# alessandroragano/nomad

Measured on AMD Instinct MI355X. Metric: clips/sec embedded + NxM NOMAD distances, 16kHz x 4s batches, higher is better.
Workload: dtype f32

## Files before the change

### nomad_amd/csrc/nomad_ctx.hip.h

```cpp
#pragma once
#include <hip/hip_runtime.h>

#include <algorithm>
#include <cmath>
#include <cstdarg>
#include <cstdio>
#include <cstdlib>
#include <cstring>
#include <atomic>
#include <mutex>
#include <string>
#include <vector>

#include "../../include/nomad_hip.h"

#include "dtypes.hip.h"
#include "gemm_f32.hip.h"

#define NOMAD_INTERNAL __attribute__((visibility("hidden")))

using namespace nomad;

inline thread_local char g_err[512] = "";

namespace {

int fail(int code, const char* fmt, ...) {
    va_list ap;
    va_start(ap, fmt);
    vsnprintf(g_err, sizeof(g_err), fmt, ap);
    va_end(ap);
    return code;
}

#define HIP_TRY(expr)                                                                        \
    do {                                                                                     \
        hipError_t _e = (expr);                                                              \
        if (_e != hipSuccess) return fail(NOMAD_ERR_HIP, "%s: %s", #expr, hipGetErrorString(_e)); \
    } while (0)

constexpr int kConvK[7] = {10, 3, 3, 3, 3, 2, 2};
constexpr int kConvS[7] = {5, 2, 2, 2, 2, 2, 2};
constexpr int kSplitKLayersMaxM = 4096;
constexpr size_t kSplitKPartFloats = (size_t)4 * 512 * 64 * 64;
constexpr long long kPairScratchDoubles = 1 << 21;
constexpr int kEventChunk = 8192;
const int* const kNoInts = nullptr;
const hipStream_t kNoStream = reinterpret_cast<hipStream_t>(~uintptr_t(0));

}

struct LayerDev {
    float *qkv_w, *qkv_b, *o_w, *o_b, *ln1_w, *ln1_b, *fc1_w, *fc1_b, *fc2_w, *fc2_b, *ln2_w, *ln2_b;
};


struct Tuning {
    bool splitk_lnb_fuse = true;
    bool splitk_ln_fuse = true;
    bool splitk_posconv = true;
    bool splitk_layers = true;
    bool f32_plain_epi = true;
    bool f32_lean = true, f32_direct_epi = true, f32_skew = true, f32_res_ahead = true;
    int f32_mixed = 1;
    int f32_mixed_m1 = 0;
    int f32_mixed_slots = 0;
    double f32_mixed_min = 0.05, f32_mixed_max = 0.70;
    bool f32_mixed_prefer = false;
    bool f32_quant_tile = true;
    double f32_quant_penalty = 0.0;
    bool f32_longk_33 = false;
    int f32_mid_tile = 31;
    bool f32_attn_vt4 = true;
    bool f32_attn_struct_loads = false;
    bool bf16_posconv_slab = true;
    int bf16_attn_dma = 2;
    int bf16_attn_v3 = 2;
    int bf16_attn_tail = 0;
    int bf16_ln_rows = 4;
    bool bf16_conv0_mfma = true;
    bool bf16_conv0_gelu_erf = false;
    int p8_min_tiles = 256;
    bool p8_nt_stores = true;
    int p8_rpre = 3;
    bool x3_plain_epi = true;
    bool p8_three_b = true;
    int p8_n192 = 0;
    bool p9 = true;
    bool p9_res = true;
    bool p9_share = false;
    bool p9_tail_split = false;
    int p9_short = 1;
    bool attn_bwd_small = true;
    bool p9_wl = false;
    bool p9_late = true;
    int p9_skew = 0;
    int concurrent_parts = 1;
};

#ifdef NOMAD_DIAG
static void tuning_from_env(Tuning& t) {
    auto geti = [](const char* n, int d) { const char* e = getenv(n); return e ? atoi(e) : d; };
    auto getb = [](const char* n, bool d) { const char* e = getenv(n); return e ? atoi(e) != 0 : d; };
    auto getd = [](const char* n, double d) { const char* e = getenv(n); return e ? atof(e) : d; };
    t.splitk_ln_fuse = getb("NOMAD_SPLITK_LN", t.splitk_ln_fuse);
    t.splitk_posconv = getb("NOMAD_SPLITK_POSCONV", t.splitk_posconv);
    t.splitk_layers = getb("NOMAD_SPLITK_LAYERS", t.splitk_layers);
    t.f32_plain_epi = getb("NOMAD_F32_PLAIN_EPI", t.f32_plain_epi);
    t.f32_lean = getb("NOMAD_F32_LEAN", t.f32_lean);
    t.f32_direct_epi = getb("NOMAD_F32_DIRECT_EPI", t.f32_direct_epi);
    t.f32_skew = getb("NOMAD_F32_SKEW", t.f32_skew);
    t.f32_res_ahead = getb("NOMAD_F32_RES_AHEAD", t.f32_res_ahead);
    t.f32_mixed = geti("NOMAD_F32_MIXED", t.f32_mixed);
    t.f32_mixed_m1 = geti("NOMAD_F32_MIXED_M1", t.f32_mixed_m1);
    t.f32_mixed_slots = geti("NOMAD_F32_MIXED_SLOTS", t.f32_mixed_slots);
    t.f32_mixed_min = getd("NOMAD_F32_MIXED_MIN", t.f32_mixed_min);
    t.f32_mixed_max = getd("NOMAD_F32_MIXED_MAX", t.f32_mixed_max);
    t.f32_mixed_prefer = getb("NOMAD_F32_MIXED_PREFER", t.f32_mixed_prefer);
    t.f32_quant_tile = getb("NOMAD_F32_QUANT_TILE", t.f32_quant_tile);
    t.f32_quant_penalty = getd("NOMAD_F32_QUANT_PENALTY", t.f32_quant_penalty);
    t.f32_longk_33 = getb("NOMAD_F32_LONGK_33", t.f32_longk_33);
    t.f32_mid_tile = geti("NOMAD_F32_MID_TILE", t.f32_mid_tile);
    t.bf16_attn_dma = geti("NOMAD_BF16_ATTN_DMA", t.bf16_attn_dma);
    t.f32_attn_struct_loads = geti("NOMAD_F32_ATTN_STRUCT_LOADS", t.f32_attn_struct_loads) != 0;
    t.bf16_posconv_slab = geti("NOMAD_BF16_POSCONV_SLAB", t.bf16_posconv_slab) != 0;
    t.bf16_attn_v3 = geti("NOMAD_BF16_ATTN_V3", t.bf16_attn_v3);
    t.bf16_attn_tail = geti("NOMAD_BF16_ATTN_TAIL", t.bf16_attn_tail);
    t.bf16_ln_rows = geti("NOMAD_BF16_LN_ROWS", t.bf16_ln_rows);
    t.bf16_conv0_mfma = getb("NOMAD_BF16_CONV0_MFMA", t.bf16_conv0_mfma);
    t.p8_min_tiles = geti("NOMAD_BF16_8PHASE_MIN_TILES", t.p8_min_tiles);
    t.p8_nt_stores = getb("NOMAD_BF16_NT_STORES", t.p8_nt_stores);
    t.p8_rpre = geti("NOMAD_BF16_RPRE", t.p8_rpre);
    t.x3_plain_epi = getb("NOMAD_X3_PLAIN_EPI", t.x3_plain_epi);
    t.p8_three_b = getb("NOMAD_BF16_B3", t.p8_three_b);
    t.p8_n192 = geti("NOMAD_BF16_N192", t.p8_n192);
    t.p9 = getb("NOMAD_BF16_P9", t.p9);
    t.p9_tail_split = getb("NOMAD_BF16_P9_TAIL", t.p9_tail_split);
    t.p9_share = getb("NOMAD_BF16_P9_SHARE", t.p9_share);
    t.p9_res = getb("NOMAD_BF16_P9_RES", t.p9_res);
    t.p9_short = geti("NOMAD_BF16_P9_SHORT", t.p9_short);
    t.p9_skew = geti("NOMAD_BF16_P9_SKEW", t.p9_skew);
    t.p9_late = getb("NOMAD_BF16_P9_LATE", t.p9_late);
    t.p9_wl = getb("NOMAD_BF16_P9_WL", t.p9_wl);
    t.splitk_lnb_fuse = getb("NOMAD_SPLITK_LNB", t.splitk_lnb_fuse);
    t.f32_attn_vt4 = getb("NOMAD_F32_ATTN_VT4", t.f32_attn_vt4);
    t.bf16_conv0_gelu_erf = getb("NOMAD_BF16_CONV0_GELU_ERF", t.bf16_conv0_gelu_erf);
    t.attn_bwd_small = getb("NOMAD_ATTN_BWD_SMALL", t.attn_bwd_small);
}
#endif

struct nomad_ctx {
    int device = 0;
    int num_cus = 256;
    Tuning tune;
    bool keep = false;
    float* conv0_w = nullptr;
    float* conv_w[7] = {};
    float *gn_w = nullptr, *gn_b = nullptr, *fln_w = nullptr, *fln_b = nullptr;
    float *proj_w = nullptr, *proj_b = nullptr;
    float *pos_w = nullptr, *pos_b = nullptr;
    float *eln_w = nullptr, *eln_b = nullptr;
    LayerDev layers[NOMAD_NUM_LAYERS] = {};
    float *emb_w = nullptr, *emb_b = nullptr;
    float* splitk_part = nullptr;
    float* splitk_cur = nullptr;
    bool splitk_ok = false;
    struct PendingLn {
        const float* gamma = nullptr;
        const float* beta = nullptr;
        float* out = nullptr;
        float* out2 = nullptr;
        bool armed = false, done = false;
// ... 86 lines not shown
        c->p_fl[cls] += flops;
        c->p_n[cls] += 1;
        if (cls2 >= 0) {
            c->p_fl[cls2] += flops;
            c->p_n[cls2] += 1;
        }
        slot = c->ev_used;
        c->ev_class[slot / 2] = cls | ((cls2 + 1) << 8);
        c->ev_used += 2;
        (void)hipEventRecord(c->ev[slot], s);
    }
    ~Scope() {
        if (slot >= 0) (void)hipEventRecord(c->ev[slot + 1], s);
    }
};

RowMap plain_map(int M, int ld) { return RowMap{0, 0, M > 0 ? M : 1, ld}; }

int occ_pad(int occ, int lds) {
    if (occ <= 0) return 0;
    const int budget = (160 * 1024 / occ) & ~255;
    return budget > lds ? budget - lds : 0;
}

GemmParams dense(const float* A, int lda, const float* W, const float* bias, const float* R, float* C, int M, int N,
                 int K, int gelu) {
    GemmParams p{};
    p.A = A;
    p.amap = plain_map(M, lda);
    p.kchunk = K;
    p.kstride = 0;
    p.W = W;
    p.ldw = K;
    p.C = C;
    p.cmap = plain_map(M, N);
    p.bias = bias;
    p.R = R;
    p.rmap = plain_map(M, N);
    p.M = M;
    p.N = N;
    p.K = K;
    p.n_valid = N;
    p.gelu = gelu;
    return p;
}

}

NOMAD_INTERNAL int run_gemm(nomad_ctx* c, GemmParams p, int groups, int tile, hipStream_t s, int occ = 0);
NOMAD_INTERNAL int gemm_f32_dispatch(nomad_ctx* c, GemmParams p, int groups, int tile, hipStream_t s, int occ);
NOMAD_INTERNAL hipError_t gemm_f32_n48_split(const GemmParams& q, int groups, hipStream_t s, int S);
NOMAD_INTERNAL int pick_tile(const nomad_ctx* c, int M, int N, int K);
NOMAD_INTERNAL int mixed_split_rows(const nomad_ctx* c, int M, int N);
NOMAD_INTERNAL int run_gemm_bf16(nomad_ctx* c, GemmParams p, int groups, hipStream_t s, int tile = -1);
#ifdef NOMAD_DIAG
NOMAD_INTERNAL int gemm_f32_timeline_read(unsigned long long* out_host, int n);
NOMAD_INTERNAL int gemm_bf16_timeline_read(unsigned long long* out_host, int n);
#endif
```

### nomad_amd/csrc/nomad_gemm_f32.hip

```cpp
#include "nomad_ctx.hip.h"

int gemm_f32_dispatch(nomad_ctx* c, GemmParams p, int groups, int tile, hipStream_t s, int occ) {
    if (tile == 29 && occ == 0) occ = 4;
    const double flops = 2.0 * p.M * (double)p.n_valid * p.K * groups;
    Scope sc(c, s, NOMAD_K_GEMM, flops, tile == 33 ? NOMAD_K_GEMM_BIG : ((tile == 34 || tile == 31 || tile == 48) ? NOMAD_K_GEMM_FINE : -1));
    hipError_t e;
    if (c->gemm_x3 && tile == 48 && p.N == 64)
        tile = 37;
    if (c->gemm_x3 && (tile == 31 || tile == 34 || tile == 37) && p.N % 128 == 0 &&
        (long long)((p.M + 127) / 128) * (p.N / 128) >= 512)
        tile = 20;
    const bool plain_cr = c->tune.f32_plain_epi && p.c_colblk == 0 && p.cmap.clip_rows >= p.M && !p.cmap.pref &&
                          (!p.R || (p.rmap.clip_rows >= p.M && !p.rmap.pref)) && (!p.DG || (p.dgmap.clip_rows >= p.M && !p.dgmap.pref));
    if (c->gemm_x3 && plain_cr && (tile == 20 || tile == 31 || tile == 34 || tile == 37)) {
        constexpr int T = 16 | 32;
        switch (tile) {
            case 20: e = launch_gemm_glds<128, 128, 32, 2, 2, 2, false, 12 | T, true>(p, groups, s, occ_pad(occ, GldsCfg<128, 128, 32, 2, 2>::LDS_BYTES)); break;
            case 31: e = launch_gemm_glds<128, 128, 32, 4, 2, 2, false, 12 | T, true>(p, groups, s, occ_pad(occ, GldsCfg<128, 128, 32, 4, 2>::LDS_BYTES)); break;
            case 34: e = launch_gemm_glds<128, 64, 32, 4, 2, 3, false, 12 | T, true>(p, groups, s); break;
            default: e = launch_gemm_glds<64, 64, 32, 2, 2, 3, false, 12 | T, true>(p, groups, s); break;
        }
        if (e != hipSuccess) return fail(NOMAD_ERR_HIP, "gemm (bf16x3 products) launch: %s", hipGetErrorString(e));
        return 0;
    }
    if (c->gemm_x3 && (tile == 20 || tile == 31 || tile == 33 || tile == 34 || tile == 37)) {
        switch (tile) {
            case 20: e = launch_gemm_glds<128, 128, 32, 2, 2, 2, false, 12, true>(p, groups, s, occ_pad(occ, GldsCfg<128, 128, 32, 2, 2>::LDS_BYTES)); break;
            case 31: e = launch_gemm_glds<128, 128, 32, 4, 2, 2, false, 12, true>(p, groups, s, occ_pad(occ, GldsCfg<128, 128, 32, 4, 2>::LDS_BYTES)); break;
            case 33: e = launch_gemm_glds<256, 128, 16, 4, 2, 3, false, 13, true>(p, groups, s); break;
            case 34: e = launch_gemm_glds<128, 64, 32, 4, 2, 3, false, 12, true>(p, groups, s); break;
            default: e = launch_gemm_glds<64, 64, 32, 2, 2, 3, false, 12, true>(p, groups, s); break;
        }
        if (e != hipSuccess) return fail(NOMAD_ERR_HIP, "gemm (bf16x3 products) launch: %s", hipGetErrorString(e));
        return 0;
    }
    if (plain_cr && (tile == 33 || tile == 31 || tile == 37 || tile == 34 || tile == 20)) {
        constexpr int P = 16, T = 16 | 32;
        const bool tr = p.Upre || p.DG;
        const int variants = (c->tune.f32_lean ? 1 : 0) | (c->tune.f32_direct_epi ? 2 : 0) | (c->tune.f32_skew ? 4 : 0) | (c->tune.f32_res_ahead ? 8 : 0);
        const bool lean = (variants & 1) && !tr && !p.amap.pref && p.group_m == 0 && p.kchunk >= p.K &&
                          (p.amap.clip_rows >= p.M || p.amap.clip_rows >= 2);
        const bool direct = lean && (variants & 2) && !p.R && p.n_valid == p.N;
        const bool skew = lean && (variants & 4);
        const bool ahead = lean && (variants & 8) && p.R && !p.gelu && p.n_valid == p.N && p.rmap.clip_rows >= p.M;
        constexpr int L = 16384, D = 1024, S = 64, RA = 32768;
        if (lean && skew && tile == 33 && groups == 1 && (p.R ? ahead : direct)) {
            const int m1 = mixed_split_rows(c, p.M, p.N);
            if (m1 > 0) {
                e = p.R ? launch_gemm_mixed<13 | P | L | S | RA, 13 | P | L | S | RA>(p, m1, s)
                        : launch_gemm_mixed<13 | P | L | S | D, 13 | P | L | S | D>(p, m1, s);
                if (e != hipSuccess) return fail(NOMAD_ERR_HIP, "gemm launch: %s", hipGetErrorString(e));
                return 0;
            }
// ... 208 lines not shown
        if (R) HIP_TRY((launch_gemm_mixed<V | 32768, V | 32768>(pp, m1, st)));
        else HIP_TRY((launch_gemm_mixed<V | 1024, V | 1024>(pp, m1, st)));
        return 0;
    }
    if (tile == 97 || tile == 98) {
        if (N % 128 || K % 32 || gelu || !R) return fail(NOMAD_ERR_INVALID, "nomad_diag_gemm: tile %d needs N %% 128 == 0, K %% 32 == 0, a residual and no GELU", tile);
        GemmParams pp = dense(A, K, W, bias, R, C, M, N, K, gelu);
        hipStream_t st = static_cast<hipStream_t>(stream);
        Scope sc(c, st, NOMAD_K_GEMM, 2.0 * M * (double)N * K, NOMAD_K_GEMM_BIG);
        if (tile == 97) HIP_TRY((launch_gemm_glds<256, 128, 16, 4, 2, 3, false, 13 | 16 | 64 | 16384 | 32768>(pp, 1, st)));
        else HIP_TRY((launch_gemm_glds<128, 128, 32, 4, 2, 2, false, 12 | 16 | 16384 | 32768>(pp, 1, st, occ_pad(0, GldsCfg<128, 128, 32, 4, 2>::LDS_BYTES))));
        return 0;
    }
    if (tile >= 88 && tile <= 93) {
        if (N % 128 || K % 32) return fail(NOMAD_ERR_INVALID, "nomad_diag_gemm: N %% 128 or K %% 32 != 0");
        GemmParams pp = dense(A, K, W, bias, R, C, M, N, K, gelu);
        hipStream_t st = static_cast<hipStream_t>(stream);
        Scope sc(c, st, NOMAD_K_GEMM, 2.0 * M * (double)N * K, NOMAD_K_GEMM_BIG);
        constexpr int L = 16384;
        switch (tile) {
            case 88: HIP_TRY((launch_gemm_glds<256, 128, 16, 4, 2, 3, false, 13 | 16 | L>(pp, 1, st))); break;
            case 89: HIP_TRY((launch_gemm_glds<256, 128, 16, 4, 2, 3, false, 13 | 16 | 1024 | L>(pp, 1, st))); break;
            case 90: HIP_TRY((launch_gemm_glds<256, 128, 16, 4, 2, 3, false, 13 | 16 | 64 | 1024 | L>(pp, 1, st))); break;
            case 91: HIP_TRY((launch_gemm_glds<256, 128, 16, 4, 2, 3, false, 13 | 16 | 64 | L>(pp, 1, st))); break;
            case 92: HIP_TRY((launch_gemm_glds<128, 128, 32, 4, 2, 2, false, 12 | 16 | L>(pp, 1, st, occ_pad(0, GldsCfg<128, 128, 32, 4, 2>::LDS_BYTES)))); break;
            default: HIP_TRY((launch_gemm_glds<128, 128, 32, 4, 2, 2, false, 12 | 16 | 1024 | L>(pp, 1, st, occ_pad(0, GldsCfg<128, 128, 32, 4, 2>::LDS_BYTES)))); break;
        }
        return 0;
    }
    if (tile == 84 || tile == 85) {
        if (N % 128 || K % 16) return fail(NOMAD_ERR_INVALID, "nomad_diag_gemm: N %% 128 or K %% 16 != 0");
        GemmParams pp = dense(A, K, W, bias, R, C, M, N, K, gelu);
        Scope sc(c, static_cast<hipStream_t>(stream), NOMAD_K_GEMM, 2.0 * M * (double)N * K, NOMAD_K_GEMM_BIG);
        if (tile == 85) return fail(NOMAD_ERR_INVALID, "nomad_diag_gemm: tile 85 (BK = 8) went with the 16x16x4 products (16-deep k groups)");
        HIP_TRY((launch_gemm_glds<256, 128, 16, 4, 2, 3, false, 13 | 16 | 64 | 1024>(pp, 1, static_cast<hipStream_t>(stream))));
        return 0;
    }
    if (tile == 82 || tile == 83 || tile == 87 || tile == 96) {
        if (N % 128 || K % 16 || K < 64) return fail(NOMAD_ERR_INVALID, "nomad_diag_gemm: persistent kernel needs N %% 128 == 0, K %% 16 == 0, K >= 64");
        GemmParams pp = dense(A, K, W, bias, R, C, M, N, K, gelu);
        Scope sc(c, static_cast<hipStream_t>(stream), NOMAD_K_GEMM, 2.0 * M * (double)N * K, NOMAD_K_GEMM_BIG);
        HIP_TRY(launch_gemm_pers(pp, static_cast<hipStream_t>(stream), c->num_cus, tile == 83, tile == 87, tile == 96));
        return 0;
    }
    if (tile < 0 || (tile > 47 && (tile < 60 || tile > 81) && tile != 86)) return fail(NOMAD_ERR_INVALID, "nomad_diag_gemm: tile id %d", tile);
    const int bn = (tile == 46 || tile == 47) ? 64 : tile >= 60 ? (tile == 67 ? 256 : 128) : kBN[tile], bk = tile == 46 ? 32 : tile == 47 ? 16 : tile >= 60 ? (tile == 73 ? 32 : 16) : kBK[tile];
    if (N % bn || K % bk) return fail(NOMAD_ERR_INVALID, "nomad_diag_gemm: N %% %d or K %% %d != 0", bn, bk);
    GemmParams p = dense(A, K, W, bias, R, C, M, N, K, gelu);
    p.group_m = group_m;
    return run_gemm(c, p, 1, tile, static_cast<hipStream_t>(stream), occ);
}

}
```

### nomad_amd/csrc/nomad_hip.hip

```cpp
#include "nomad_ctx.hip.h"

#include "attention.hip.h"
#include "attention_bf16_v2.hip.h"
#include "attention_bf16_v3.hip.h"
#include "posconv_bf16_slab.hip.h"
#include "attention_f32_v2.hip.h"
#include "attention_bwd.hip.h"
#include "backward.hip.h"
#include "frontend.hip.h"
#include "gemm_bf16.hip.h"
#include "gemm_bf16_8phase.hip.h"
#include "gemm_bf16_p9.hip.h"
#include "gemm_bf16x3.hip.h"
#include "gemm_f32.hip.h"
#ifdef NOMAD_DIAG
#endif
#include "pairwise.hip.h"
#include "rowops.hip.h"
#include "train.hip.h"
#include "wav_reader.h"

namespace {

struct Shapes {
// ... 274 lines not shown
    const long long count4 = (long long)p.M * p.N / 4;
    hipLaunchKernelGGL(splitk_epilogue_kernel, dim3((unsigned)((count4 + 255) / 256)), dim3(256), 0, s,
                       reinterpret_cast<const float4*>(c->splitk_cur), S, count4, p.N / 4, reinterpret_cast<const float4*>(p.bias),
                       reinterpret_cast<const float4*>(p.R), reinterpret_cast<float4*>(p.C), p.gelu);
    HIP_TRY(hipGetLastError());
    return 0;
}

static bool posconv_splitk_applies(const nomad_ctx* c, const GemmParams& p, int groups, int tile) {
    if (!c->tune.splitk_posconv || !c->splitk_ok || !c->splitk_cur || groups != 16 || tile != 48) return false;
    if (p.DG || p.K != 6144 || p.kchunk != p.K || p.n_valid != 48 || p.c_goff != 48) return false;
    const bool c_plain = p.cmap.clip_rows >= p.M && p.cmap.off == 0 && p.cmap.ld == 768;
    return c_plain && (long long)((p.M + 255) / 256) * 16 < 256 && (size_t)4 * p.M * 768 <= kSplitKPartFloats;
}

static int run_posconv_splitk(nomad_ctx* c, const GemmParams& p, hipStream_t s) {
    constexpr int S = 4;
    GemmParams q = p;
    q.K = p.K / S;
    q.kchunk = q.K;
    q.a_soff = q.K;
    q.w_soff = q.K;
    q.C = c->splitk_cur;
    q.cmap = plain_map(p.M, 768);
    q.c_soff = (long long)p.M * 768;
    q.bias = nullptr;
    q.R = nullptr;
    q.Upre = nullptr;
    q.gelu = 0;
    {
        Scope sc(c, s, NOMAD_K_GEMM, 2.0 * p.M * 48.0 * p.K * 16, NOMAD_K_GEMM_FINE);
        HIP_TRY(gemm_f32_n48_split(q, 16, s, S));
    }
    Scope sc(c, s, NOMAD_K_ROW, 0.0);
    hipLaunchKernelGGL(posconv_splitk_epilogue_kernel, dim3(p.M), dim3(192), 0, s, c->splitk_cur, S, p.M, p.bias, p.R, p.rmap, p.r_goff, p.Upre, p.C,
                       p.gelu);
    HIP_TRY(hipGetLastError());
    return 0;
}

}

int run_gemm(nomad_ctx* c, GemmParams p, int groups, int tile, hipStream_t s, int occ) {
    {
        int S = 0;
        if (splitk_applies(c, p, groups, tile, &S)) return run_gemm_splitk(c, p, S, s);
        if (posconv_splitk_applies(c, p, groups, tile)) return run_posconv_splitk(c, p, s);
    }
    return gemm_f32_dispatch(c, p, groups, tile, s, occ);
}

namespace {


int run_layernorm(nomad_ctx* c, const float* in, const float* g, const float* b, float* out, float* out2, int M, int N,
                  hipStream_t s) {
    Scope sc(c, s, NOMAD_K_ROW, 0.0);
    const int blocks = (M + 3) / 4;
    if (N == 768) hipLaunchKernelGGL((layernorm_kernel<3, float, float>), dim3(blocks), dim3(256), 0, s, in, g, b, out, out2, M);
    else if (N == 512) hipLaunchKernelGGL((layernorm_kernel<2, float, float>), dim3(blocks), dim3(256), 0, s, in, g, b, out, out2, M);
    else return fail(NOMAD_ERR_INVALID, "layernorm: N=%d unsupported", N);
    HIP_TRY(hipGetLastError());
    return 0;
}

template <typename TIn>
int run_head(nomad_ctx* c, const TIn* x, int B, int T, const float* w, const float* b, float* emb, const int* tpref,
             float* pool, hipStream_t s) {
    Scope sc(c, s, NOMAD_K_ROW, 2.0 * B * 768 * 256);
    hipLaunchKernelGGL(head_pool_kernel<TIn>, dim3((T + kHeadChunk - 1) / kHeadChunk, B), dim3(256), 0, s, x, tpref ? 0 : T, pool, tpref);
    hipLaunchKernelGGL(head_kernel, dim3(B), dim3(1024), 0, s, pool, tpref ? 0 : T, w, b, emb, tpref);
    HIP_TRY(hipGetLastError());
    return 0;
}

DropCfg make_drop(const nomad_ctx* c, float p) {
    DropCfg d{};
    d.seed_lo = (uint32_t)c->drop_seed;
    d.seed_hi = (uint32_t)(c->drop_seed >> 32);
    const double t = (double)p * 4294967296.0;
    d.threshold = p <= 0.f ? 0u : (t >= 4294967295.0 ? 4294967295u : (uint32_t)(t + 0.5));
    d.scale = 1.0f / (1.0f - p);
    return d;
}


int run_attention(nomad_ctx* c, const float* qkv, float* out, float* lse, int B, int T, hipStream_t s,
                  const DropCfg* dc = nullptr, uint32_t site = 0, int bh0 = 0) {
    const double flops = 4.0 * B * 12.0 * (double)T * T * 64;
    Scope sc(c, s, NOMAD_K_ATTN, flops);
    const dim3 grid((T + 63) / 64, B * 12);
    if (dc && dc->threshold)
        hipLaunchKernelGGL((attention_f32_kernel<float, true>), grid, dim3(256), 0, s, qkv, out, lse, T, kNoInts, *dc, site, bh0);
    else if (T >= kAttnV2MinT)
    {
#ifdef NOMAD_DIAG
        if (c->tune.f32_attn_struct_loads) HIP_TRY(launch_attention_f32_v2<false>(qkv, out, lse, B, T, kNoInts, s));
        else if (!c->tune.f32_attn_vt4) HIP_TRY((launch_attention_f32_v2<true, false>(qkv, out, lse, B, T, kNoInts, s)));
        else
#endif
            HIP_TRY(launch_attention_f32_v2(qkv, out, lse, B, T, kNoInts, s));
    }
    else
        hipLaunchKernelGGL((attention_f32_kernel<float, false>), grid, dim3(256), 0, s, qkv, out, lse, T, kNoInts, DropCfg{}, 0u, 0);
    HIP_TRY(hipGetLastError());
    return 0;
// ... 237 lines not shown
}

}

static int forward_impl(nomad_ctx* c, const float* wav, int B, int n_samples, const float* head_w, const float* head_b,
                        float* emb, float* layers_out, void* workspace, size_t workspace_bytes, nomad_stream_t stream,
                        const Saved* sv) {
    Shapes sh;
    if (!c || !wav || !emb || !workspace || B <= 0 || !make_shapes(B, n_samples, &sh))
        return fail(NOMAD_ERR_INVALID, "nomad_embed: bad argument (B=%d, n_samples=%d)", B, n_samples);
    const Layout lay = make_layout(sh, c->keep);
    if (workspace_bytes < lay.total)
        return fail(NOMAD_ERR_WORKSPACE, "nomad_embed: workspace %zu < required %zu", workspace_bytes, lay.total);
    hipStream_t s = static_cast<hipStream_t>(stream);
    char* ws = static_cast<char*>(workspace);
    auto F = [&](size_t off) { return reinterpret_cast<float*>(ws + off); };
    const int T = sh.T, M = sh.M;
    float* const loss_block = (sv == nullptr && layers_out != nullptr && lay.splitk != 0 && c->tune.splitk_layers) ? F(lay.splitk) : nullptr;
    const SplitKScope splitk(c, (sv != nullptr || loss_block != nullptr) && !c->train_ready);
    float* const prev_cur = c->splitk_cur;
    c->splitk_cur = sv != nullptr ? c->splitk_part : loss_block;
    struct CurRestore { nomad_ctx* c; float* v; ~CurRestore() { c->splitk_cur = v; } } cur_restore{c, prev_cur};
    int rc;
    const bool reg = sv != nullptr;
    const DropCfg d_in = make_drop(c, reg ? c->p_input : 0.f), d_res = make_drop(c, reg ? c->p_drop : 0.f),
                  d_att = make_drop(c, reg ? c->p_attn : 0.f);
    int nbr = 1;
    unsigned bmask[4] = {reg ? c->layer_mask : 0xFFFu, 0xFFFu, 0xFFFu, 0xFFFu};
    if (reg && c->branches > 1) {
        if (B % c->branches) return fail(NOMAD_ERR_INVALID, "nomad_embed_train: B=%d is not %d equal branches", B, c->branches);
        nbr = c->branches;
        for (int i = 0; i < nbr; ++i) bmask[i] = c->branch_mask[i];
    }
    const long long act = (long long)M * 768;

    double* stats = reinterpret_cast<double*>(ws + lay.stats);
    float* gn_scale = sv ? sv->gn_scale : F(lay.scale);
    float* gn_shift = sv ? sv->gn_shift : F(lay.shift);
    {
        Scope sc(c, s, NOMAD_K_FRONT, 0.0);
        launch_wav_stats(wav, n_samples, sh.L[0], sh.L[0], B, stats, kNoInts, s);
        hipLaunchKernelGGL(gn_fold_kernel, dim3(B), dim3(512), 0, s, stats, c->conv0_w, c->gn_w, c->gn_b, sh.L[0],
                           gn_scale, gn_shift, sv ? sv->gn_mean : nullptr, sv ? sv->gn_rstd : nullptr, kNoInts);
    }
    {
        Scope sc(c, s, NOMAD_K_FRONT, 2.0 * B * (double)sh.L[0] * 512 * 10);
        hipLaunchKernelGGL(conv0_gn_gelu_kernel<float>, dim3((sh.L[0] + kConv0Frames - 1) / kConv0Frames, B), dim3(256), 0, s,
                           wav, n_samples, sh.L[0], c->conv0_w, gn_scale, gn_shift, F(lay.conv[0]), kNoInts, kNoInts);
    }
    HIP_TRY(hipGetLastError());

    for (int i = 1; i < 7; ++i) {
        const int k = kConvK[i];
        GemmParams p{};
        p.A = F(lay.conv[i - 1]);
        p.amap = RowMap{0, (long long)sh.L[i - 1] * 512, sh.L[i], kConvS[i] * 512};
        p.K = k * 512;
        p.kchunk = p.K;
        p.W = c->conv_w[i];
        p.ldw = p.K;
        p.C = (sv && i == 6) ? sv->c6 : F(lay.conv[i]);
        p.Upre = sv ? sv->u[i] : nullptr;
        p.M = B * sh.L[i];
        p.N = 512;
        p.n_valid = 512;
        p.cmap = plain_map(p.M, 512);
        p.rmap = p.cmap;
        p.gelu = 1;
        if ((rc = run_gemm(c, p, 1, pick_tile(c, p.M, 512, p.K), s))) return rc;
    }

    if ((rc = run_layernorm(c, sv ? sv->c6 : F(lay.conv[6]), c->fln_w, c->fln_b, F(lay.featln), nullptr, M, 512, s)))
        return rc;
    float* xpad = F(lay.xpad);
    const long long grp_stride = (long long)B * (T + 128) * 48;
    const RowMap pad_map{64LL * 48, (long long)(T + 128) * 48, T, 48};
    {
        Scope sc(c, s, NOMAD_K_ROW, 0.0);
        hipLaunchKernelGGL(zero_pad_rows_kernel<float>, dim3(16 * B), dim3(256), 0, s, xpad, T, kNoInts, kNoInts, B);
    }
    {
        GemmParams p = dense(F(lay.featln), 512, c->proj_w, c->proj_b, nullptr, xpad, M, 768, 512, 0);
        p.cmap = pad_map;
        p.c_colblk = 48;
        p.c_colblk_stride = grp_stride;
        if ((rc = run_gemm(c, p, 1, pick_tile(c, M, 768, 512), s))) return rc;
    }
    if (d_in.threshold) {
        Scope sc(c, s, NOMAD_K_ROW, 0.0);
        hipLaunchKernelGGL(dropout_groups_kernel, dim3(M), dim3(192), 0, s, xpad, T, grp_stride, d_in, kSiteInput);
    }
    {
        GemmParams p{};
        p.A = xpad;
        p.amap = RowMap{0, (long long)(T + 128) * 48, T, 48};
        p.a_goff = grp_stride;
        p.K = 6144;
        p.kchunk = 6144;
        p.W = c->pos_w;
        p.ldw = 6144;
        p.w_goff = 64LL * 6144;
        p.bias = c->pos_b;
        p.bias_goff = 48;
        p.C = sv ? sv->y0 : F(lay.y);
        p.Upre = sv ? sv->upc : nullptr;
        p.cmap = plain_map(M, 768);
// ... 49 lines not shown
        arm_ln(d.ln1_w, d.ln1_b, x2s, nullptr);
        if ((rc = run_gemm(c, dense(ctxb, 768, d.o_w, d.o_b, d_res.threshold ? nullptr : xs, y1, Ms, 768, 768, 0), 1,
                           pick_tile(c, Ms, 768, 768), s))) {
            c->pending_ln = {};
            return rc;
        }
        if (d_res.threshold && (rc = run_dropout(c, y1, xs, y1, acts, d_res, site_proj(l), s, idx0))) return rc;
        if ((rc = ln_after(y1, d.ln1_w, d.ln1_b, x2s, nullptr))) return rc;
        {
            GemmParams p = dense(x2s, 768, d.fc1_w, d.fc1_b, nullptr, hs, Ms, 3072, 768, 1);
            p.Upre = sv ? sv->L[l].u + r0 * 3072 : nullptr;
            if ((rc = run_gemm(c, p, 1, pick_tile(c, Ms, 3072, 768), s))) return rc;
        }
        arm_ln(d.ln2_w, d.ln2_b, xs, lo);
        if ((rc = run_gemm(c, dense(hs, 3072, d.fc2_w, d.fc2_b, d_res.threshold ? nullptr : x2s, y2, Ms, 768, 3072, 0), 1,
                           pick_tile(c, Ms, 768, 3072), s))) {
            c->pending_ln = {};
            return rc;
        }
        if (d_res.threshold && (rc = run_dropout(c, y2, x2s, y2, acts, d_res, site_ffn(l), s, idx0))) return rc;
        return ln_after(y2, d.ln2_w, d.ln2_b, xs, lo);
    };
    for (int l = 0; l < NOMAD_NUM_LAYERS; ++l) {
        unsigned all = 1u, any = 0u;
        for (int br = 0; br < nbr; ++br) {
            all &= (bmask[br] >> l) & 1u;
            any |= (bmask[br] >> l) & 1u;
        }
        if (all) {
            if ((rc = run_layer(l, 0, B))) return rc;
            continue;
        }
        for (int br = 0; br < nbr; ++br) {
            const int c0 = br * (B / nbr), nc = B / nbr;
            if ((bmask[br] >> l) & 1u) {
                if ((rc = run_layer(l, c0, nc))) return rc;
            } else if (layers_out) {
                const long long r0 = (long long)c0 * T;
                HIP_TRY(hipMemcpyAsync(layers_out + (size_t)l * M * 768 + r0 * 768, x + r0 * 768,
                                       sizeof(float) * (size_t)nc * T * 768, hipMemcpyDeviceToDevice, s));
            }
        }
        (void)any;
    }

    return run_head<float>(c, x, B, T, head_w ? head_w : c->emb_w, head_b ? head_b : c->emb_b, emb, kNoInts, F(lay.h), s);
}

struct RaggedShapes {
    int B = 0, max_l0 = 0, max_t = 0, min_t = 1 << 30;
    long long rows[7] = {};
    long long P = 0;
    long long blocks = 0;
    std::vector<int> meta;
    size_t off_lens() const { return 0; }
    size_t off_pref(int i) const { return (size_t)B + (size_t)i * (B + 1); }
    size_t off_ppref() const { return (size_t)B + (size_t)7 * (B + 1); }
    size_t off_bpref() const { return (size_t)B + (size_t)8 * (B + 1); }
};

static bool make_ragged(int B, const int* lens, RaggedShapes* r) {
    r->B = B;
    r->meta.assign((size_t)B + 9 * (size_t)(B + 1), 0);
    for (int c = 0; c < B; ++c) {
        Shapes sh;
        if (!make_shapes(1, lens[c], &sh)) return false;
        r->meta[c] = lens[c];
        for (int i = 0; i < 7; ++i) {
            r->meta[r->off_pref(i) + c + 1] = r->meta[r->off_pref(i) + c] + sh.L[i];
            r->rows[i] += sh.L[i];
        }
        r->meta[r->off_ppref() + c + 1] = r->meta[r->off_ppref() + c] + sh.T + 128;
        r->P += sh.T + 128;
        const int nb = (sh.T + kPosBlk - 1) / kPosBlk;
        r->meta[r->off_bpref() + c + 1] = r->meta[r->off_bpref() + c] + nb;
        r->blocks += nb;
        r->max_l0 = sh.L[0] > r->max_l0 ? sh.L[0] : r->max_l0;
        r->max_t = sh.T > r->max_t ? sh.T : r->max_t;
        r->min_t = sh.T < r->min_t ? sh.T : r->min_t;
    }
    return r->rows[0] < (1LL << 31) / 512 * 256;
}

struct RaggedLayout {
    size_t meta, stats, scale, shift, conva, convb, xpad, x, x2, y, qkv, ctxb, h, total;
};

static RaggedLayout make_ragged_layout(const RaggedShapes& r) {
    RaggedLayout l{};
    size_t off = 0;
    auto take = [&](size_t bytes) {
        size_t o = off;
        off += align_up(bytes);
        return o;
    };
    const size_t M = (size_t)r.rows[6];
    l.meta = take(sizeof(int) * r.meta.size());
    l.stats = take(sizeof(double) * stats_doubles(r.B, r.max_l0));
    l.scale = take(sizeof(float) * 512 * r.B);
    l.shift = take(sizeof(float) * 512 * r.B);
    l.conva = take(sizeof(float) * 512 * (size_t)r.rows[0]);
    l.convb = take(sizeof(float) * 512 * (size_t)r.rows[1]);
    l.xpad = take(sizeof(float) * 768 * (size_t)r.P);
    l.x = take(sizeof(float) * 768 * M);
    l.x2 = take(sizeof(float) * 768 * M);
    l.y = take(sizeof(float) * 768 * M);
    l.qkv = take(sizeof(float) * 2304 * M);
    l.ctxb = take(sizeof(float) * 768 * M);
    l.h = take(sizeof(float) * 3072 * M);
    l.total = off;
    return l;
}

static int forward_ragged(nomad_ctx* c, const float* wav, int B, int stride, const int* lens_host, const float* head_w,
                          const float* head_b, float* emb, void* workspace, size_t workspace_bytes,
                          nomad_stream_t stream) {
    RaggedShapes rs;
    if (!c || !wav || !lens_host || !emb || !workspace || B <= 0 || !make_ragged(B, lens_host, &rs))
        return fail(NOMAD_ERR_INVALID, "nomad_embed_ragged: bad argument (B=%d)", B);
    for (int i = 0; i < B; ++i)
        if (lens_host[i] > stride) return fail(NOMAD_ERR_INVALID, "nomad_embed_ragged: clip %d longer than the row stride", i);
    const RaggedLayout lay = make_ragged_layout(rs);
    if (workspace_bytes < lay.total)
        return fail(NOMAD_ERR_WORKSPACE, "nomad_embed_ragged: workspace %zu < required %zu", workspace_bytes, lay.total);
    hipStream_t s = static_cast<hipStream_t>(stream);
    char* ws = static_cast<char*>(workspace);
    auto F = [&](size_t off) { return reinterpret_cast<float*>(ws + off); };
    int* meta = reinterpret_cast<int*>(ws + lay.meta);
    std::vector<int>& staged = c->ragged_meta_ring[c->ragged_seq++ & 3];
    staged = rs.meta;
    HIP_TRY(hipMemcpyAsync(meta, staged.data(), sizeof(int) * rs.meta.size(), hipMemcpyHostToDevice, s));
    const int* lens = meta + rs.off_lens();
    auto pref = [&](int i) { return static_cast<const int*>(meta + rs.off_pref(i)); };
    const int* tpref = pref(6);
    const int* ppref = meta + rs.off_ppref();
    const int M = (int)rs.rows[6];
    int rc;

    double* stats = reinterpret_cast<double*>(ws + lay.stats);
    float *scale = F(lay.scale), *shift = F(lay.shift);
    float* cb[2] = {F(lay.conva), F(lay.convb)};
    {
        Scope sc(c, s, NOMAD_K_FRONT, 0.0);
        launch_wav_stats(wav, stride, 0, rs.max_l0, B, stats, lens, s);
        hipLaunchKernelGGL(gn_fold_kernel, dim3(B), dim3(512), 0, s, stats, c->conv0_w, c->gn_w, c->gn_b, 0, scale, shift,
                           static_cast<float*>(nullptr), static_cast<float*>(nullptr), lens);
    }
    {
        Scope sc(c, s, NOMAD_K_FRONT, 2.0 * (double)rs.rows[0] * 512 * 10);
        hipLaunchKernelGGL(conv0_gn_gelu_kernel<float>, dim3((rs.max_l0 + kConv0Frames - 1) / kConv0Frames, B), dim3(256), 0,
                           s, wav, stride, 0, c->conv0_w, scale, shift, cb[0], lens, pref(0));
    }
    for (int i = 1; i < 7; ++i) {
        GemmParams p{};
        p.A = cb[(i - 1) % 2];
        p.amap = RowMap{0, 0, 0, kConvS[i] * 512, pref(i), pref(i - 1), B, 512};
        p.K = kConvK[i] * 512;
        p.kchunk = p.K;
        p.W = c->conv_w[i];
        p.ldw = p.K;
        p.C = cb[i % 2];
        p.M = (int)rs.rows[i];
        p.N = 512;
        p.n_valid = 512;
        p.cmap = plain_map(p.M, 512);
        p.rmap = p.cmap;
        p.gelu = 1;
        if ((rc = run_gemm(c, p, 1, pick_tile(c, p.M, 512, p.K), s))) return rc;
    }
    float* featln = cb[1];
    if ((rc = run_layernorm(c, cb[0], c->fln_w, c->fln_b, featln, nullptr, M, 512, s))) return rc;
    float* xpad = F(lay.xpad);
    const long long grp_stride = rs.P * 48;
    const RowMap pad_map{64LL * 48, 0, 0, 48, tpref, ppref, B, 48};
    {
        Scope sc(c, s, NOMAD_K_ROW, 0.0);
        hipLaunchKernelGGL(zero_pad_rows_kernel<float>, dim3(16 * B), dim3(256), 0, s, xpad, 0, tpref, ppref, B);
    }
    {
        GemmParams p = dense(featln, 512, c->proj_w, c->proj_b, nullptr, xpad, M, 768, 512, 0);
        p.cmap = pad_map;
        p.c_colblk = 48;
        p.c_colblk_stride = grp_stride;
        if ((rc = run_gemm(c, p, 1, pick_tile(c, M, 768, 512), s))) return rc;
    }
    float *x = F(lay.x), *x2 = F(lay.x2), *y = F(lay.y), *qkv = F(lay.qkv), *ctxb = F(lay.ctxb), *hbuf = F(lay.h);
    {
        GemmParams p{};
        p.A = xpad;
        p.amap = RowMap{0, 0, 0, 48, tpref, ppref, B, 48};
        p.a_goff = grp_stride;
        p.K = 6144;
        p.kchunk = 6144;
        p.W = c->pos_w;
        p.ldw = 6144;
        p.w_goff = 64LL * 6144;
        p.bias = c->pos_b;
        p.bias_goff = 48;
        p.C = y;
        p.cmap = plain_map(M, 768);
        p.c_goff = 48;
        p.R = xpad;
        p.rmap = pad_map;
        p.r_goff = grp_stride;
        p.M = M;
        p.N = 64;
// ... 2202 lines not shown
```

Before: 2422.

## Add Winograd-style paired-output kernel for stride-2 k=3 feature convolutions

Adds a dedicated f32 MFMA kernel for the stride-2, kernel-3 conv layers of the feature extractor. Each pair of adjacent outputs is computed with shared and differenced input/weight terms, cutting the effective reduction length per pair from two full 1536-wide dot products to 2560 terms. The kernel fuses GELU into the epilogue and supports both uniform and ragged batches, using new per-clip pair prefix metadata. It is on by default unless the bf16x3 path is active, and it replaces a tuned generic GEMM with a new hand-scheduled kernel.

```diff
diff --git a/nomad_amd/csrc/conv_s2_f32.hip.h b/nomad_amd/csrc/conv_s2_f32.hip.h
--- /dev/null
+++ b/nomad_amd/csrc/conv_s2_f32.hip.h
@@ -0,0 +1,234 @@
+#pragma once
+#include "gemm_f32.hip.h"
+
+namespace nomad {
+
+struct ConvS2Params {
+    const float* X;
+    const float* W;
+    float* Y;
+    float* Upre;
+    int pairs;
+    int tiles_m;
+    int L, Lin, ppc;
+    unsigned ppc_magic;
+    int ppc_shift;
+    const int* pp;
+    const int* opref;
+    const int* ipref;
+    int nclips;
+};
+
+struct ConvS2Cfg {
+    static constexpr int BMP = 128, BN = 128, NT = 512;
+    static constexpr int STAGE = 8 * 1024 + 132;
+    static constexpr int ZOFF = 8 * 1024;
+    static constexpr int LDS_BYTES = 2 * STAGE * 4;
+};
+
+struct PairRows {
+    long long in0, in_last, out0;
+    bool odd_ok;
+};
+
+template <bool RAGGED>
+__device__ __forceinline__ PairRows conv_s2_pair(const ConvS2Params& p, int s) {
+    PairRows r;
+    if (RAGGED) {
+        int lo = 0, hi = p.nclips;
+        while (hi - lo > 1) {
+            const int mid = (lo + hi) >> 1;
+            if (p.pp[mid] <= s) lo = mid;
+            else hi = mid;
+        }
+        const int j = s - p.pp[lo];
+        const int L = p.opref[lo + 1] - p.opref[lo];
+        r.in0 = (long long)p.ipref[lo] + 4 * j;
+        r.in_last = (long long)p.ipref[lo + 1] - 1;
+        r.out0 = (long long)p.opref[lo] + 2 * j;
+        r.odd_ok = 2 * j + 1 < L;
+    } else {
+        const int c = p.ppc_magic ? fast_div(s, p.ppc_magic, p.ppc_shift) : (p.ppc == 1 ? s : 0);
+        const int j = s - c * p.ppc;
+        r.in0 = (long long)c * p.Lin + 4 * j;
+        r.in_last = (long long)c * p.Lin + p.Lin - 1;
+        r.out0 = (long long)c * p.L + 2 * j;
+        r.odd_ok = 2 * j + 1 < p.L;
+    }
+    return r;
+}
+
+template <bool RAGGED>
+__global__ __launch_bounds__(512, 4) void conv_s2_f32_kernel(const ConvS2Params p) {
+    using Cfg = ConvS2Cfg;
+    extern __shared__ __attribute__((aligned(16))) float smem[];
+    const int tid = threadIdx.x, lane = tid & 63;
+    const int wave = __builtin_amdgcn_readfirstlane(tid >> 6);
+    const int wm = wave >> 1, wn = wave & 1;
+    const int nwg = p.tiles_m * 4;
+    const int wg = xcd_remap(blockIdx.x, nwg);
+    const int tile_m = wg >> 2, tile_n = wg & 3;
+    const int m0 = tile_m * Cfg::BMP, n0 = tile_n * Cfg::BN;
+
+    if (tid < 2 * 33) *reinterpret_cast<f32x4*>(smem + (tid / 33) * Cfg::STAGE + Cfg::ZOFF + (tid % 33) * 4) = (f32x4){0.f, 0.f, 0.f, 0.f};
+
+    const long long tile_in0 = conv_s2_pair<RAGGED>(p, m0).in0;
+    const float* const a_tile = uniform_ptr(p.X + tile_in0 * 512);
+    const float* const b_tile = uniform_ptr(p.W + (long long)n0 * 1536);
+    int v1a, v1b;
+    {
+        const int r1 = tid >> 2, lc = (tid & 3) ^ ((r1 >> 2) & 3);
+        const int s = min(m0 + r1, p.pairs - 1);
+        const PairRows pr = conv_s2_pair<RAGGED>(p, s);
+        v1a = (int)(((pr.in0 + 2 - tile_in0) * 512 + lc * 4) * 4);
+        v1b = (r1 * 1536 + lc * 4) * 4;
+    }
+    const int f0 = wave >> 2;
+    int v2a[3], v2b;
+    {
+        const int r = (tid & 255) >> 1, lc = (tid & 1) ^ ((r >> 3) & 1);
+        const int s = min(m0 + r, p.pairs - 1);
+        const PairRows pr = conv_s2_pair<RAGGED>(p, s);
+#pragma unroll
+        for (int i = 0; i < 3; ++i) {
+            const int f = i == 2 ? 4 : f0 + 2 * i;
+            const long long row = min(pr.in0 + f, pr.in_last);
+            v2a[i] = (int)(((row - tile_in0) * 512 + lc * 4) * 4);
+        }
+        v2b = (r * 1536 + lc * 4) * 4;
+    }
+    auto issue = [&](const int q, const int buf) {
+        float* st = smem + buf * Cfg::STAGE + wave * 256;
+        if (q < 32) {
+            const int k0 = q * 16;
+            dma16_buffer(a_tile, (lptr_t)(st), v1a, k0 * 4);
+            dma16_buffer(b_tile, (lptr_t)(st + 2048), v1b, k0 * 4);
+            dma16_buffer(b_tile, (lptr_t)(st + 4096), v1b, (k0 + 1024) * 4);
+        } else {
+            const int k0 = (q - 32) * 8;
+            dma16_buffer(a_tile, (lptr_t)(st), v2a[0], k0 * 4);
+            dma16_buffer(a_tile, (lptr_t)(st + 2048), v2a[1], k0 * 4);
+            if (f0 == 0) dma16_buffer(a_tile, (lptr_t)(st + 4096), v2a[2], k0 * 4);
+            else dma16_buffer(b_tile, (lptr_t)(st + 4096), v2b, k0 * 4);
+            dma16_buffer(b_tile, (lptr_t)(st + 6144), v2b, ((1 + f0) * 512 + k0) * 4);
+        }
+    };
+
+    const int fi = lane & 15, g = lane >> 4;
+    const int ra = wm * 32 + fi, rb = wn * 64 + fi;
+    const int sw1 = (g ^ ((fi >> 2) & 3)) * 4;
+    const int o1a = ra * 16 + sw1, o1b = 2048 + rb * 16 + sw1;
+    const int sw2 = ((g & 1) ^ (fi >> 3)) * 4;
+    const bool lo = g < 2;
+    const int oEF = (lo ? 0 : 1024) + ra * 8 + sw2;
+    const int oES = lo ? 2048 + ra * 8 + sw2 : Cfg::ZOFF;
+    const int oOF = (lo ? 3072 : 4096) + ra * 8 + sw2;
+    const int oOS = lo ? Cfg::ZOFF : 2048 + ra * 8 + sw2;
+    const int oBE = (lo ? 5120 : 6144) + rb * 8 + sw2;
+    const int oBO = (lo ? 6144 : 7168) + rb * 8 + sw2;
+
+    f32x4 E[2][4], O[2][4];
+#pragma unroll
+    for (int si = 0; si < 2; ++si)
+#pragma unroll
+        for (int sj = 0; sj < 4; ++sj) E[si][sj] = (f32x4){0.f, 0.f, 0.f, 0.f};
+
+    auto rd = [&](const float* base, int off) { return *reinterpret_cast<const f32x4*>(base + off); };
+    auto mm = [&](f32x4 (&acc)[2][4], const f32x4 (&a)[2], const f32x4 (&b)[4]) {
+#pragma unroll
+        for (int c = 0; c < 4; ++c)
+#pragma unroll
+            for (int si = 0; si < 2; ++si)
+#pragma unroll
+                for (int sj = 0; sj < 4; ++sj) acc[si][sj] = __builtin_amdgcn_mfma_f32_16x16x4f32(b[sj][c], a[si][c], acc[si][sj], 0, 0, 0);
+    };
+    auto step1 = [&](const float* st) {
+        f32x4 a[2], b[4];
+#pragma unroll
+        for (int si = 0; si < 2; ++si) a[si] = rd(st, o1a + si * 256);
+#pragma unroll
+        for (int sj = 0; sj < 4; ++sj) {
+            const f32x4 u = rd(st, o1b + sj * 256), v = rd(st, o1b + 2048 + sj * 256);
+#pragma unroll
+            for (int e = 0; e < 4; ++e) b[sj][e] = u[e] + v[e];
+        }
+        mm(E, a, b);
+    };
+    auto operand = [&](const float* st, int of, int os, f32x4 (&a)[2]) {
+#pragma unroll
+        for (int si = 0; si < 2; ++si) {
+            const f32x4 u = rd(st, of + si * 128), v = rd(st, os + si * 128);
+#pragma unroll
+            for (int e = 0; e < 4; ++e) a[si][e] = u[e] - v[e];
+        }
+    };
+    auto step2 = [&](const float* st) {
+        f32x4 a[2], b[4];
+        operand(st, oEF, oES, a);
+#pragma unroll
+        for (int sj = 0; sj < 4; ++sj) b[sj] = rd(st, oBE + sj * 128);
+        mm(E, a, b);
+        asm volatile("" ::: "memory");
+        __builtin_amdgcn_sched_barrier(0);
+        operand(st, oOF, oOS, a);
+#pragma unroll
+        for (int sj = 0; sj < 4; ++sj) b[sj] = rd(st, oBO + sj * 128);
+        mm(O, a, b);
+    };
+
+    auto wait_step = [] {
+        asm volatile("s_waitcnt vmcnt(0)" ::: "memory");
+        __syncthreads();
+    };
+    float* const st0 = smem;
+    float* const st1 = smem + Cfg::STAGE;
+    issue(0, 0);
+    for (int q = 0; q < 32; q += 2) {
+        wait_step();
+        issue(q + 1, 1);
+        step1(st0);
+        wait_step();
+        issue(q + 2, 0);
+        step1(st1);
+    }
+#pragma unroll
+    for (int si = 0; si < 2; ++si)
+#pragma unroll
+        for (int sj = 0; sj < 4; ++sj) O[si][sj] = E[si][sj];
+    for (int q = 32; q < 96; q += 2) {
+        wait_step();
+        issue(q + 1, 1);
+        step2(st0);
+        wait_step();
+        if (q + 2 < 96) issue(q + 2, 0);
+        step2(st1);
+    }
+
+    int lane_e = lane;
+    asm volatile("" : "+v"(lane_e));
+    const int col = n0 + wn * 64 + 4 * (lane_e >> 4);
+#pragma unroll
+    for (int si = 0; si < 2; ++si) {
+        const int s = m0 + wm * 32 + (lane_e & 15) + 16 * si;
+        if (s >= p.pairs) continue;
+        const PairRows pr = conv_s2_pair<RAGGED>(p, s);
+        const long long ie = pr.out0 * 512 + col, io = ie + 512;
+#pragma unroll
+        for (int sj = 0; sj < 4; ++sj) {
+            f32x4 ve = E[si][sj], vo = O[si][sj];
+            if (p.Upre) {
+                *reinterpret_cast<f32x4*>(p.Upre + ie + sj * 16) = ve;
+                if (pr.odd_ok) *reinterpret_cast<f32x4*>(p.Upre + io + sj * 16) = vo;
+            }
+#pragma unroll
+            for (int e = 0; e < 4; ++e) {
+                ve[e] = gelu_erf(ve[e]);
+                vo[e] = gelu_erf(vo[e]);
+            }
+            *reinterpret_cast<f32x4*>(p.Y + ie + sj * 16) = ve;
+            if (pr.odd_ok) *reinterpret_cast<f32x4*>(p.Y + io + sj * 16) = vo;
+        }
+    }
+}
+
+}
diff --git a/nomad_amd/csrc/nomad_ctx.hip.h b/nomad_amd/csrc/nomad_ctx.hip.h
--- a/nomad_amd/csrc/nomad_ctx.hip.h
+++ b/nomad_amd/csrc/nomad_ctx.hip.h
@@ -68,6 +68,7 @@
     double f32_mixed_min = 0.05, f32_mixed_max = 0.70;
     bool f32_mixed_prefer = false;
     bool f32_quant_tile = true;
+    bool f32_conv_wino = true;
     double f32_quant_penalty = 0.0;
     bool f32_longk_33 = false;
     int f32_mid_tile = 31;
@@ -118,6 +119,7 @@
     t.f32_mixed_max = getd("NOMAD_F32_MIXED_MAX", t.f32_mixed_max);
     t.f32_mixed_prefer = getb("NOMAD_F32_MIXED_PREFER", t.f32_mixed_prefer);
     t.f32_quant_tile = getb("NOMAD_F32_QUANT_TILE", t.f32_quant_tile);
+    t.f32_conv_wino = getb("NOMAD_F32_CONV_WINO", t.f32_conv_wino);
     t.f32_quant_penalty = getd("NOMAD_F32_QUANT_PENALTY", t.f32_quant_penalty);
     t.f32_longk_33 = getb("NOMAD_F32_LONGK_33", t.f32_longk_33);
     t.f32_mid_tile = geti("NOMAD_F32_MID_TILE", t.f32_mid_tile);
@@ -310,6 +312,8 @@
 NOMAD_INTERNAL hipError_t gemm_f32_n48_split(const GemmParams& q, int groups, hipStream_t s, int S);
 NOMAD_INTERNAL int pick_tile(const nomad_ctx* c, int M, int N, int K);
 NOMAD_INTERNAL int mixed_split_rows(const nomad_ctx* c, int M, int N);
+NOMAD_INTERNAL int run_conv_s2_f32(nomad_ctx* c, const float* X, const float* W, float* Y, float* Upre, int B, int Lin, int L,
+                                   const int* pp, const int* opref, const int* ipref, int pairs, hipStream_t s);
 NOMAD_INTERNAL int run_gemm_bf16(nomad_ctx* c, GemmParams p, int groups, hipStream_t s, int tile = -1);
 #ifdef NOMAD_DIAG
 NOMAD_INTERNAL int gemm_f32_timeline_read(unsigned long long* out_host, int n);
diff --git a/nomad_amd/csrc/nomad_gemm_f32.hip b/nomad_amd/csrc/nomad_gemm_f32.hip
--- a/nomad_amd/csrc/nomad_gemm_f32.hip
+++ b/nomad_amd/csrc/nomad_gemm_f32.hip
@@ -1,4 +1,5 @@
 #include "nomad_ctx.hip.h"
+#include "conv_s2_f32.hip.h"
 
 int gemm_f32_dispatch(nomad_ctx* c, GemmParams p, int groups, int tile, hipStream_t s, int occ) {
     if (tile == 29 && occ == 0) occ = 4;
@@ -313,3 +314,72 @@
 }
 
 }
+
+int run_conv_s2_f32(nomad_ctx* c, const float* X, const float* W, float* Y, float* Upre, int B, int Lin, int L, const int* pp,
+                    const int* opref, const int* ipref, int pairs, hipStream_t s) {
+    ConvS2Params p{};
+    p.X = X;
+    p.W = W;
+    p.Y = Y;
+    p.Upre = Upre;
+    p.pairs = pairs;
+    p.tiles_m = (pairs + ConvS2Cfg::BMP - 1) / ConvS2Cfg::BMP;
+    p.nclips = B;
+    if (ipref) {
+        p.pp = pp;
+        p.opref = opref;
+        p.ipref = ipref;
+    } else {
+        p.L = L;
+        p.Lin = Lin;
+        p.ppc = (L + 1) / 2;
+        if (Lin < 2 * L + 1 || pairs != B * p.ppc) return fail(NOMAD_ERR_INVALID, "conv_s2: %d clips of %d -> %d frames, %d pairs", B, Lin, L, pairs);
+        p.ppc_magic = 0;
+        p.ppc_shift = 0;
+        if (B > 1 && p.ppc > 1) fast_div_magic((unsigned)p.ppc, &p.ppc_magic, &p.ppc_shift);
+    }
+    const double flops = 2.0 * (double)pairs * 512 * 2560;
+    Scope sc(c, s, NOMAD_K_GEMM, flops, NOMAD_K_GEMM_BIG);
+    static LdsAttrOnce attr_u, attr_r;
+    hipError_t e;
+    if (ipref) {
+        if ((e = attr_r.ensure(reinterpret_cast<const void*>(conv_s2_f32_kernel<true>), ConvS2Cfg::LDS_BYTES)) != hipSuccess)
+            return fail(NOMAD_ERR_HIP, "conv_s2 attribute: %s", hipGetErrorString(e));
+        hipLaunchKernelGGL(conv_s2_f32_kernel<true>, dim3(p.tiles_m * 4), dim3(ConvS2Cfg::NT), ConvS2Cfg::LDS_BYTES, s, p);
+    } else {
+        if ((e = attr_u.ensure(reinterpret_cast<const void*>(conv_s2_f32_kernel<false>), ConvS2Cfg::LDS_BYTES)) != hipSuccess)
+            return fail(NOMAD_ERR_HIP, "conv_s2 attribute: %s", hipGetErrorString(e));
+        hipLaunchKernelGGL(conv_s2_f32_kernel<false>, dim3(p.tiles_m * 4), dim3(ConvS2Cfg::NT), ConvS2Cfg::LDS_BYTES, s, p);
+    }
+    if ((e = hipGetLastError()) != hipSuccess) return fail(NOMAD_ERR_HIP, "conv_s2 launch: %s", hipGetErrorString(e));
+    return 0;
+}
+
+#ifdef NOMAD_DIAG
+extern "C" {
+int nomad_diag_conv_s2(nomad_ctx* c, const float* X, const float* W, float* Y, float* U, int B, const int* lin_host, int ragged,
+                       void* stream) {
+    if (!c || !X || !W || !Y || !lin_host || B <= 0) return fail(NOMAD_ERR_INVALID, "nomad_diag_conv_s2: bad argument");
+    std::vector<int> meta(3 * (size_t)(B + 1), 0);
+    for (int b = 0; b < B; ++b) {
+        const int lin = lin_host[b], L = lin >= 3 ? (lin - 3) / 2 + 1 : 0;
+        if (L <= 0 || (!ragged && lin != lin_host[0])) return fail(NOMAD_ERR_INVALID, "nomad_diag_conv_s2: clip %d of %d frames", b, lin);
+        meta[b + 1] = meta[b] + (L + 1) / 2;
+        meta[(B + 1) + b + 1] = meta[(B + 1) + b] + L;
+        meta[2 * (B + 1) + b + 1] = meta[2 * (B + 1) + b] + lin;
+    }
+    hipStream_t s = static_cast<hipStream_t>(stream);
+    int* d = nullptr;
+    HIP_TRY(hipMalloc(&d, sizeof(int) * meta.size()));
+    int rc = 0;
+    if (hipMemcpy(d, meta.data(), sizeof(int) * meta.size(), hipMemcpyHostToDevice) != hipSuccess) rc = fail(NOMAD_ERR_HIP, "nomad_diag_conv_s2: copy");
+    const int lin0 = lin_host[0], L0 = (lin0 - 3) / 2 + 1;
+    if (rc == 0)
+        rc = ragged ? run_conv_s2_f32(c, X, W, Y, U, B, 0, 0, d, d + (B + 1), d + 2 * (B + 1), meta[B], s)
+                    : run_conv_s2_f32(c, X, W, Y, U, B, lin0, L0, nullptr, nullptr, nullptr, meta[B], s);
+    if (rc == 0 && hipStreamSynchronize(s) != hipSuccess) rc = fail(NOMAD_ERR_HIP, "nomad_diag_conv_s2: kernel");
+    (void)hipFree(d);
+    return rc;
+}
+}
+#endif
diff --git a/nomad_amd/csrc/nomad_hip.hip b/nomad_amd/csrc/nomad_hip.hip
--- a/nomad_amd/csrc/nomad_hip.hip
+++ b/nomad_amd/csrc/nomad_hip.hip
@@ -350,6 +350,8 @@
 
 namespace {
 
+bool conv_wino(const nomad_ctx* c, int i) { return c->tune.f32_conv_wino && !c->gemm_x3 && kConvK[i] == 3 && kConvS[i] == 2; }
+
 
 int run_layernorm(nomad_ctx* c, const float* in, const float* g, const float* b, float* out, float* out2, int M, int N,
                   hipStream_t s) {
@@ -693,6 +695,12 @@
 
     for (int i = 1; i < 7; ++i) {
         const int k = kConvK[i];
+        if (conv_wino(c, i)) {
+            if ((rc = run_conv_s2_f32(c, F(lay.conv[i - 1]), c->conv_w[i], F(lay.conv[i]), sv ? sv->u[i] : nullptr, B, sh.L[i - 1], sh.L[i],
+                                      nullptr, nullptr, nullptr, B * ((sh.L[i] + 1) / 2), s)))
+                return rc;
+            continue;
+        }
         GemmParams p{};
         p.A = F(lay.conv[i - 1]);
         p.amap = RowMap{0, (long long)sh.L[i - 1] * 512, sh.L[i], kConvS[i] * 512};
@@ -848,16 +856,18 @@
     long long rows[7] = {};
     long long P = 0;
     long long blocks = 0;
+    long long pairs[5] = {};
     std::vector<int> meta;
     size_t off_lens() const { return 0; }
     size_t off_pref(int i) const { return (size_t)B + (size_t)i * (B + 1); }
     size_t off_ppref() const { return (size_t)B + (size_t)7 * (B + 1); }
     size_t off_bpref() const { return (size_t)B + (size_t)8 * (B + 1); }
+    size_t off_pairpref(int i) const { return (size_t)B + (size_t)(8 + i) * (B + 1); }
 };
 
 static bool make_ragged(int B, const int* lens, RaggedShapes* r) {
     r->B = B;
-    r->meta.assign((size_t)B + 9 * (size_t)(B + 1), 0);
+    r->meta.assign((size_t)B + 13 * (size_t)(B + 1), 0);
     for (int c = 0; c < B; ++c) {
         Shapes sh;
         if (!make_shapes(1, lens[c], &sh)) return false;
@@ -865,6 +875,10 @@
         for (int i = 0; i < 7; ++i) {
             r->meta[r->off_pref(i) + c + 1] = r->meta[r->off_pref(i) + c] + sh.L[i];
             r->rows[i] += sh.L[i];
+        }
+        for (int i = 1; i <= 4; ++i) {
+            r->meta[r->off_pairpref(i) + c + 1] = r->meta[r->off_pairpref(i) + c] + (sh.L[i] + 1) / 2;
+            r->pairs[i] += (sh.L[i] + 1) / 2;
         }
         r->meta[r->off_ppref() + c + 1] = r->meta[r->off_ppref() + c] + sh.T + 128;
         r->P += sh.T + 128;
@@ -948,6 +962,12 @@
                            s, wav, stride, 0, c->conv0_w, scale, shift, cb[0], lens, pref(0));
     }
     for (int i = 1; i < 7; ++i) {
+        if (conv_wino(c, i)) {
+            if ((rc = run_conv_s2_f32(c, cb[(i - 1) % 2], c->conv_w[i], cb[i % 2], nullptr, B, 0, 0, meta + rs.off_pairpref(i), pref(i),
+                                      pref(i - 1), (int)rs.pairs[i], s)))
+                return rc;
+            continue;
+        }
         GemmParams p{};
         p.A = cb[(i - 1) % 2];
         p.amap = RowMap{0, 0, 0, kConvS[i] * 512, pref(i), pref(i - 1), B, 512};
```

New measurement: 2508, median of 6. 3.5% higher.
